# icyveins7/pydsproutines

Measured on AMD Instinct MI355X. Metric: CAF Msamples/s (4k template x 256 freq bins), higher is better.
Workload: dtype f32

## Files before the change

### pydsproutines_amd/csrc/caf_fused.hip

```cpp
#include <algorithm>
#include <cstdlib>
#include <type_traits>

#include "caf_internal.h"
#include "caf_fft_dev.h"
#include "caf_wave.h"

namespace caf {

constexpr int FB = 16384;
constexpr int FP_P1 = 4384;
constexpr int FP_IM = 16 * FP_P1;
constexpr int F_LDS_BYTES = 2 * FP_IM;
constexpr int F_LDS_DATA = F_LDS_BYTES / 8;
__host__ __device__ constexpr int fp_row2(int n2) { return ((n2 >> 1) & 3) * 1088 + ((n2 & 1) + 2 * (n2 >> 3)) * 256; }
static_assert(fp_row2(15) + 256 <= FP_P1 && FP_P1 % 256 == 32, "planar image geometry");

#define CAF_AS1 __attribute__((address_space(1)))
#define CAF_AS4 __attribute__((address_space(4)))
typedef float v2f_t __attribute__((ext_vector_type(2)));
typedef float v4f_t __attribute__((ext_vector_type(4)));
typedef int v2i_t __attribute__((ext_vector_type(2)));
__device__ __forceinline__ float2 ld2(const float2* base, uint32_t elem) {
    const uint64_t u = *reinterpret_cast<const CAF_AS1 uint64_t*>((const CAF_AS1 char*)base + (elem << 3));
// ... 96 lines not shown
__device__ __forceinline__ Tp* uniform_ptr(Tp* p) {
    const uint64_t v = reinterpret_cast<uint64_t>(p);
    const uint32_t lo = __builtin_amdgcn_readfirstlane((uint32_t)v);
    const uint32_t hi = __builtin_amdgcn_readfirstlane((uint32_t)(v >> 32));
    return reinterpret_cast<Tp*>(((uint64_t)hi << 32) | lo);
}
__device__ __forceinline__ __amdgpu_buffer_rsrc_t buf_of(const void* base, uint32_t bytes) {
    return __builtin_amdgcn_make_buffer_rsrc(const_cast<void*>(base), 0, (int)bytes, 0x00020000);
}
constexpr int CAF_AUX_SC1 = 16;
constexpr int CAF_AUX_NT = 2;
template <int MODE>
__device__ __forceinline__ void tile_store(__amdgpu_buffer_rsrc_t r, uint32_t voff, uint32_t soff, float val) {
    __builtin_amdgcn_raw_buffer_store_b32(__builtin_bit_cast(int, val), r, (int)voff, (int)soff, MODE == 1 ? (CAF_AUX_SC1 | CAF_AUX_NT) : 0);
}

struct F1Direct {
    float* out0;
    float* out1;
    const float* inv_e;
    const float* tscale;
    int64_t num_shifts;
    int32_t step, blk_abs;
    PeakRec* partial;
    int64_t ppt, shift_start;
};
template <int FT, int MODE = 0, int NV4 = 4, bool PK = false>
__device__ __forceinline__ void fused_item(float2* __restrict__ s_d, const float2* __restrict__ s_tw2,
                                           const float2* __restrict__ s_tw3,
                                           const float2* __restrict__ xb,
                                           const float2* __restrict__ hc,
                                           const int32_t* __restrict__ shifts,
                                           const float2* __restrict__ tw1,
                                           int32_t table_mode, int32_t nfreq, int32_t nhyp, int blk, int h0, int h1,
                                           int32_t tiles_per_blk, float* __restrict__ vt,
                                           int32_t* __restrict__ imax = nullptr, const F1Direct* f1 = nullptr) {
    static_assert(FT == 1024, "one radix-16 butterfly per thread and pass: 1024 threads (wave w owns plane n1 = w)");
    constexpr int BPT = 1;
    const int tid = threadIdx.x;
    const lds_char* img = (const lds_char*)s_d;
    const uint32_t img0 = __builtin_amdgcn_readfirstlane((uint32_t)(uintptr_t)img);
    const uint32_t wave_u = __builtin_amdgcn_readfirstlane((uint32_t)tid >> 6);
    const uint32_t m0_x1 = img0 + wave_u * 256u, m0_w = img0 + wave_u * (uint32_t)FP_P1;
    const uint32_t m2 = fp_m2((uint32_t)tid);
    constexpr int nv4 = NV4;
    float bv[16];
    uint32_t bi[4];
    float ge[16];
    if (MODE == 2 || MODE == 5) {
#pragma unroll
        for (int o = 0; o < 16; ++o) bv[o] = -1.f;
#pragma unroll
// ... 19 lines not shown
#pragma unroll
            for (int o = 0; o < 16; ++o) ge[o] = __builtin_sqrtf(ge[o]);
        }
    }

    uint32_t pk_d0 = 0, pk_nv = 0;
    if (PK) {
        const int n1 = tid & 15, n2 = (tid >> 4) & 15, q = tid >> 8;
        pk_d0 = (uint32_t)(((n2 >> 2) + 4 * q) * 64 + n1 + 16 * (n2 & 3));
        pk_nv = f1_bytes >> 2;
    }
    float2 w[BPT];
    const float2* xp = xb + (int64_t)blk * FB;
#pragma unroll
    for (int j = 0; j < BPT; ++j) w[j] = ld2(tw1, 1024u + m2);
    float* vt_blk = vt + (int64_t)blk * tiles_per_blk * nhyp * 64;
    const __amdgpu_buffer_rsrc_t rvt = buf_of(uniform_ptr(vt_blk), (uint32_t)tiles_per_blk * (uint32_t)nhyp * 256u);

    const float2* hrow_cur;
    uint32_t hb_cur;
    auto row_of = [&](int h) {
        if (table_mode) {
            hrow_cur = hc + (int64_t)h * FB;
            hb_cur = (uint32_t)tid;
        } else {
            const int t = h / nfreq;
            const int32_t sh = *((const CAF_AS4 int32_t*)shifts + (h - t * nfreq));
            hrow_cur = hc + (int64_t)t * FB;
            hb_cur = fp_hbase(m2, sh);
        }
    };
    float2 pr[BPT][16];
    float2 xr[BPT][16];
#pragma unroll
    for (int j = 0; j < BPT; ++j)
#pragma unroll
        for (int a = 0; a < 16; ++a) xr[j][a] = ld2(xp, 1024u * a + m2);
    row_of(h0);
#pragma unroll
    for (int j = 0; j < BPT; ++j)
#pragma unroll
        for (int a = 0; a < 16; ++a)
            pr[j][a] = cmul(xr[j][a],
                            ld2(hrow_cur, (1024u * a + hb_cur) & (FB - 1)));

    for (int h = h0; h < h1; ++h) {
        const bool more = h + 1 < h1;
        uint32_t hoff = (uint32_t)h * 256u;
        asm volatile("" : "+s"(hoff));
        int lz = 0;
        asm volatile("" : "+v"(lz));
        __amdgpu_buffer_rsrc_t f1_r0 = rvt, f1_r1 = rvt;
        float f1_ts = 0.f;
        if (MODE == 3) {
            f1_ts = *((const CAF_AS4 float*)f1->tscale + h);
            f1_r0 = buf_of(uniform_ptr(f1->out0 + (int64_t)h * f1->num_shifts + f1_rel0), f1->out0 ? f1_bytes : 0u);
            if (f1->out1)
                f1_r1 = buf_of(uniform_ptr(f1->out1 + (int64_t)h * f1->num_shifts + f1_rel0), f1_bytes);
        }
        float pk_v[4] = {-1.f, -1.f, -1.f, -1.f};
        uint32_t pk_i[4] = {0u, 0u, 0u, 0u};
        if (MODE == 4) {
            f1_ts = __builtin_sqrtf(*((const CAF_AS4 float*)f1->tscale + h / nfreq));
// ... 79 lines not shown
        __syncthreads();
#pragma unroll
        for (int j = 0; j < BPT; ++j) {
            const int idx = tid + j * FT;
            const int n1 = idx & 15, n2 = (idx >> 4) & 15, q = idx >> 8;
            const uint32_t rd4 = fp_rd4((uint32_t)idx), rd4i = fp_im(rd4);
            __builtin_amdgcn_sched_barrier(0);
            float2 pf0, pf1, pf2, pf3;
            if (MODE < 2) {
                lds_get4c(img, rd4, rd4i, pf0, pf1, pf2, pf3);
                __builtin_amdgcn_sched_barrier(0);
#pragma unroll
                for (int a = 0; a < 16; ++a) pr[j][a] = cmul(xr[j][a], hn[j][a]);
                __builtin_amdgcn_sched_barrier(0);
            }
#pragma unroll
            for (int i = 0; i < 4; ++i) {
                uint32_t lzi = 0;
                asm volatile("" : "+v"(lzi));
                float2 a0, a1, a2, a3;
                if (MODE < 2 && i == 0)
                    a0 = pf0, a1 = pf1, a2 = pf2, a3 = pf3;
                else
                    lds_get4c(img, rd4 + 1024u * i + lzi, rd4i + 1024u * i + lzi, a0, a1, a2, a3);
                const float2 s02 = cadd(a0, a2), d02 = csub(a0, a2), s13 = cadd(a1, a3), d13 = mulj(csub(a1, a3));
#pragma unroll
                for (int n4 = 0; n4 < 4; ++n4) {
                    if (n4 >= nv4) continue;
                    const float2 yq = n4 == 0 ? cadd(s02, s13) : n4 == 1 ? cadd(d02, d13) : n4 == 2 ? csub(s02, s13) : csub(d02, d13);
                    const int tile_u = 16 * i + 64 * n4;
// ... 24 lines not shown
                        const float gq = ge[4 * i + n4] * f1_ts;
                        const v2f_t ov = {yq.x * gq, yq.y * gq};
                        const uint32_t v3 = (uint32_t)(tile_t * 64 + n1 + 16 * (n2 & 3)) << 3, s3 = (uint32_t)tile_u * 512u;
                        __builtin_amdgcn_raw_buffer_store_b64(__builtin_bit_cast(v2i_t, ov), f1_r0, (int)v3, (int)s3, CAF_AUX_NT);
                    } else if (MODE == 3) {
                        const float outv = val * (ge[4 * i + n4] * f1_ts);
                        if (PK) {
                            const bool up = ((uint32_t)(pk_d0 + (16 * i + 64 * n4) * 64) < pk_nv) & (outv > pk_v[n4]);
                            pk_v[n4] = up ? outv : pk_v[n4];
                            pk_i[n4] = up ? (uint32_t)i : pk_i[n4];
                        }
                        const uint32_t v3 = (uint32_t)(tile_t * 64 + n1 + 16 * (n2 & 3)) << 2, s3 = (uint32_t)tile_u * 256u;
                        __builtin_amdgcn_raw_buffer_store_b32(__builtin_bit_cast(int, outv), f1_r0, (int)v3, (int)s3, CAF_AUX_NT);
                        if (f1->out1)
                            __builtin_amdgcn_raw_buffer_store_b32(__builtin_bit_cast(int, outv), f1_r1, (int)v3, (int)s3, CAF_AUX_NT);
                    } else {
                        tile_store<MODE>(rvt, voff, soff, val);
                    }
                }
                __builtin_amdgcn_sched_barrier(0);
            }
            if (MODE >= 2) {
#pragma unroll
                for (int a = 2 * EH; a < 16; ++a) pr[j][a] = cmul(xr[j][a], hn[j][a]);
            }
            __builtin_amdgcn_sched_barrier(0);
        }
        if (PK) {
            float bvv = pk_v[0];
            uint32_t bq = 0, bii = pk_i[0];
#pragma unroll
            for (int n4 = 1; n4 < NV4; ++n4) {
                const bool up = pk_v[n4] > bvv;
                bvv = up ? pk_v[n4] : bvv;
                bq = up ? (uint32_t)n4 : bq;
// ... 583 lines not shown
__device__ __forceinline__ int32_t pq_load(const int32_t* p) {
    return __hip_atomic_load(p, __ATOMIC_RELAXED, __HIP_MEMORY_SCOPE_AGENT);
}
__device__ __forceinline__ const CAF_AS4 PersistParams* params_of(const PersistParams* p) {
    uint64_t v = reinterpret_cast<uint64_t>(p);
    asm volatile("" : "+s"(v));
    return reinterpret_cast<const CAF_AS4 PersistParams*>(v);
}
typedef float v4f_u_t __attribute__((ext_vector_type(4), aligned(4)));
typedef int v4i_u_t __attribute__((ext_vector_type(4), aligned(4)));

constexpr int TW_H = 32;
constexpr int TW_PITCH = TW_H + 1;
constexpr int TW_LDS = 64 * TW_PITCH;

template <bool SURF, int DS>
__device__ __forceinline__ void transpose_wave(float* __restrict__ lds, const PersistParams* pp, int z, int tile0) {
    const CAF_AS4 PersistParams* P = params_of(pp);
    const int32_t ntmpl = P->ntmpl, nfreq = P->nfreq, step = P->step, tiles_per_blk = P->tiles_per_blk;
    const int64_t num_shifts = P->num_shifts, shift_start = P->shift_start;
    const int wave_id = __builtin_amdgcn_readfirstlane((int)(threadIdx.x >> 6));
    const int lane = threadIdx.x & 63;
    float* s_w = lds + wave_id * TW_LDS;
    const int tile = tile0 + wave_id;
    if (tile >= tiles_per_blk) return;
    const int blk = P->blk0 + z;
    const int sl0 = DS == 2 ? 128 * (tile & 255) + (tile >> 8) : tile * 64;
    const int64_t rel0 = (int64_t)blk * step + sl0;
    int64_t nv = num_shifts - (int64_t)blk * step;
    if (nv > step) nv = step;
    const int nrows = sl0 < nv ? (int)min((int64_t)64, (nv - sl0 + DS - 1) / DS) : 0;
    const int64_t pidx = (int64_t)blk * tiles_per_blk + tile;
    PeakRec* partial = P->partial;
    const int64_t ppt = P->partial_per_tmpl;
    const int s4 = 4 * (lane & 15), fq = lane >> 4;
    const int nsteps = (nfreq + TW_H - 1) / TW_H;
    for (int t = 0; t < ntmpl; ++t) {
        if (nrows == 0) {
            if (lane == 0 && partial) {
                PeakRec r;
                r.v = -1.f;
                r.delay = 0x7fffffff;
                r.f = 0;
                partial[(int64_t)t * ppt + pidx] = r;
            }
            continue;
        }
        const float* vin = uniform_ptr(P->vt + (((int64_t)z * tiles_per_blk + tile) * ntmpl + t) * (int64_t)nfreq * 64);
        float* srow0 = SURF ? uniform_ptr(P->surface + ((int64_t)t * num_shifts + rel0) * nfreq) : nullptr;
        const float ts = P->tscale[t];
        const __amdgpu_buffer_rsrc_t rin = buf_of(vin, (uint32_t)nfreq * 256u);
        const __amdgpu_buffer_rsrc_t rout = buf_of(srow0, (uint32_t)(((nrows - 1) * DS + 1) * nfreq) * 4u);
        const __amdgpu_buffer_rsrc_t rie = buf_of(uniform_ptr(P->inv_e + rel0), (uint32_t)((nrows - 1) * DS + 1) * 4u);
        float g[4], bv[4];
        int32_t bi[4];
#pragma unroll
        for (int k = 0; k < 4; ++k) {
            g[k] = __builtin_bit_cast(float, __builtin_amdgcn_raw_buffer_load_b32(rie, (s4 + k) * 4 * DS, 0, 0)) * ts;
            bv[k] = -1.f;
            bi[k] = 0;
        }
        v4f_t qa[TW_H / 4], qb[TW_H / 4];
        auto load_step = [&](v4f_t(&q)[TW_H / 4], int s) {
#pragma unroll
            for (int i = 0; i < TW_H / 4; ++i)
                q[i] = __builtin_bit_cast(v4f_t, __builtin_amdgcn_raw_buffer_load_b128(rin, (fq * 64 + s4) * 4,
                                                                                       (s * TW_H + 4 * i) * 256, CAF_AUX_SC1 | CAF_AUX_NT));
        };
        const int half = lane >> 5, col = lane & 31;
        const float* srd = s_w + half * TW_PITCH + col;
        float* swr = s_w + s4 * TW_PITCH + fq;
        const int voff = (half * DS * nfreq + col) * 4;
        auto do_step = [&](v4f_t(&q)[TW_H / 4], int s) {
            const int f0 = s * TW_H;
#pragma unroll
            for (int i = 0; i < TW_H / 4; ++i) {
                const int hyp = f0 + 4 * i + fq;
                const bool hv = hyp < nfreq;
                const float x[4] = {q[i].x * g[0], q[i].y * g[1], q[i].z * g[2], q[i].w * g[3]};
#pragma unroll
                for (int k = 0; k < 4; ++k) {
                    if (SURF) swr[k * TW_PITCH + 4 * i] = x[k];
                    const bool up = hv & (x[k] > bv[k]);
                    bv[k] = up ? x[k] : bv[k];
                    bi[k] = up ? hyp : bi[k];
                }
            }
            load_step(q, s + 2);
            if (SURF) {
                __builtin_amdgcn_wave_barrier();
                const int vo = (f0 + col < nfreq) ? voff : 0x7ffffff0;
#pragma unroll
                for (int r = 0; r < 64; r += 2)
                    __builtin_amdgcn_raw_buffer_store_b32(__builtin_bit_cast(int, srd[r * TW_PITCH]), rout, vo,
                                                          (r * DS * nfreq + f0) * 4, CAF_AUX_NT);
                __builtin_amdgcn_wave_barrier();
            }
        };
        load_step(qa, 0);
        load_step(qb, 1);
        for (int s = 0; s < nsteps; s += 2) {
            do_step(qa, s);
            do_step(qb, s + 1);
        }
#pragma unroll
        for (int k = 0; k < 4; ++k) wave_argmax<32, 16>(bv[k], bi[k]);
        float* row_max = P->row_max;
        int32_t* row_arg = P->row_arg;
        float best = -1.f;
        int32_t bdel = 0x7fffffff, bfrq = 0;
        if (fq == 0) {
            const int64_t o = (int64_t)t * num_shifts + rel0 + s4 * DS;
#pragma unroll
            for (int k = 0; k < 4; ++k) {
                if (s4 + k < nrows) {
                    if (row_max) row_max[o + k * DS] = bv[k] < 0.f ? __builtin_nanf("") : bv[k];
                    if (row_arg) row_arg[o + k * DS] = bi[k];
                    if (bv[k] > best) {
                        best = bv[k];
                        bdel = s4 + k;
                        bfrq = bi[k];
                    }
                }
            }
        }
        if (partial) {
            wave_argmax<8>(best, bdel, bfrq);
            if (lane == 0) {
                PeakRec r;
                r.v = best;
                r.delay = (int32_t)(shift_start + rel0 + bdel * DS);
                r.f = bfrq;
                partial[(int64_t)t * ppt + pidx] = r;
            }
        }
// ... 196 lines not shown
    for (;;) {
        const CAF_AS4 PersistParams* P = params_of(pp);
        const int ipb = P->ipb;
        const int z = item / ipb;
        if (P->nosurf)
            reduce_wave_nosurf(pp, z, (item - z * ipb) * PQ_TILES);
        else if (P->dstride == 2) {
            if (P->nfreq == 1)
                transpose_wave_f1<2>(pp, z, (item - z * ipb) * PQ_TILES);
            else if (P->surface)
                transpose_wave<true, 2>(lds, pp, z, (item - z * ipb) * PQ_TILES);
            else
                transpose_wave<false, 2>(lds, pp, z, (item - z * ipb) * PQ_TILES);
        } else if (P->nfreq == 1)
            transpose_wave_f1<1>(pp, z, (item - z * ipb) * PQ_TILES);
        else if (P->surface)
            transpose_wave<true, 1>(lds, pp, z, (item - z * ipb) * PQ_TILES);
        else
            transpose_wave<false, 1>(lds, pp, z, (item - z * ipb) * PQ_TILES);
        if (wave_id == 0) {
            int32_t* pq = P->pq;
            const int n_fft = P->n_fft, n_tr = P->n_tr, ngroups = P->ngroups;
            int next = -1;
            const int t = __builtin_amdgcn_readfirstlane(pq_load(&pq[PQ_TR_NEXT]));
            if (t < n_tr) {
                const bool fft_left = __builtin_amdgcn_readfirstlane(pq_load(&pq[PQ_FFT_NEXT])) < n_fft;
                if (!fft_left || __builtin_amdgcn_readfirstlane(pq_load(&pq[PQ_DONE + t / ipb])) >= ngroups) {
                    int my = 0;
                    if (lane0) my = atomicAdd(&pq[PQ_TR_NEXT], 1);
                    my = __builtin_amdgcn_readfirstlane(my);
                    if (my < n_tr) {
// ... 69 lines not shown
        f1.partial = nullptr;
        f1.ppt = 0;
        f1.shift_start = 0;
        f1.inv_e = P->inv_e;
        f1.tscale = P->tscale;
        f1.num_shifts = P->num_shifts;
        f1.step = P->step;
        f1.blk_abs = P->blk0 + blk;
        const int64_t o = ((int64_t)blk * ngroups + grp) * P->tiles_per_blk * 64;
        fused_item<1024, 5, NV4>((float2*)s_d, (const float2*)s_tw2, (const float2*)s_tw3, P->xb, P->hc, P->shifts, P->tw1,
                                 P->table_mode, P->nfreq, nhyp, blk, h0, h1, P->tiles_per_blk, P->vmax + o, P->imax + o, &f1);
    } else if (KIND == 1) {
        const int64_t o = ((int64_t)blk * ngroups + grp) * P->tiles_per_blk * 64;
        fused_item<1024, 2, NV4>((float2*)s_d, (const float2*)s_tw2, (const float2*)s_tw3, P->xb, P->hc, P->shifts, P->tw1,
                            P->table_mode, P->nfreq, nhyp, blk, h0, h1, P->tiles_per_blk, P->vmax + o, P->imax + o);
    } else {
        fused_item<1024, 1, NV4>((float2*)s_d, (const float2*)s_tw2, (const float2*)s_tw3, P->xb, P->hc, P->shifts, P->tw1,
                            P->table_mode, P->nfreq, nhyp, blk, h0, h1, P->tiles_per_blk, P->vt);
    }
    __builtin_amdgcn_fence(__ATOMIC_RELEASE, "workgroup");
    __syncthreads();
    if (threadIdx.x == 0)
        __hip_atomic_fetch_add(&params_of(pp)->pq[PQ_DONE + blk], 1, __ATOMIC_RELAXED, __HIP_MEMORY_SCOPE_AGENT);
}

__device__ __forceinline__ void cq_params(const CAF_AS4 PersistParams* P, int blk, F1Direct& f1) {
    f1.out0 = P->cqf;
    f1.out1 = nullptr;
    f1.partial = nullptr;
    f1.ppt = 0;
// ... 175 lines not shown
                }
#undef CAF_FFT_ROLE2F
            } else if (__builtin_amdgcn_readfirstlane(params_of(pp)->block_log2) == 15) {
                const int tpb2 = __builtin_amdgcn_readfirstlane(params_of(pp)->tiles_per_blk);
                const bool cq = params_of(pp)->cqf != nullptr;
#define CAF_FFT_ROLE2(NN, CC) persistent_fft_item2<NN, CC>((lds_float2*)s_d, (const lds_float2*)s_tw2, (const lds_float2*)s_tw3, pp, item)
                if (tpb2 <= 256) { if (cq) CAF_FFT_ROLE2(0, true); else CAF_FFT_ROLE2(0, false); }
                else if (tpb2 <= 384) { if (cq) CAF_FFT_ROLE2(2, true); else CAF_FFT_ROLE2(2, false); }
                else { if (cq) CAF_FFT_ROLE2(4, true); else CAF_FFT_ROLE2(4, false); }
#undef CAF_FFT_ROLE2
            }
            else {
                const int kind3 = params_of(pp)->cqf ? 3
                                  : params_of(pp)->surface_t ? 5
                                  : __builtin_amdgcn_readfirstlane(params_of(pp)->f1_direct) ? (params_of(pp)->partial ? 4 : 2)
                                  : __builtin_amdgcn_readfirstlane(params_of(pp)->nosurf) ? 1 : 0;
                const int tpb = __builtin_amdgcn_readfirstlane(params_of(pp)->tiles_per_blk);
#define CAF_FFT_ROLE(K, Q) persistent_fft_item<K, Q>((lds_float2*)s_d, (const lds_float2*)s_tw2, (const lds_float2*)s_tw3, pp, item)
                if (tpb <= 128) {
                    if (kind3 == 5) CAF_FFT_ROLE(5, 2); else if (kind3 == 4) CAF_FFT_ROLE(4, 2); else if (kind3 == 3) CAF_FFT_ROLE(3, 2); else if (kind3 == 2) CAF_FFT_ROLE(2, 2); else if (kind3 == 1) CAF_FFT_ROLE(1, 2); else CAF_FFT_ROLE(0, 2);
                } else if (tpb <= 192) {
                    if (kind3 == 5) CAF_FFT_ROLE(5, 3); else if (kind3 == 4) CAF_FFT_ROLE(4, 3); else if (kind3 == 3) CAF_FFT_ROLE(3, 3); else if (kind3 == 2) CAF_FFT_ROLE(2, 3); else if (kind3 == 1) CAF_FFT_ROLE(1, 3); else CAF_FFT_ROLE(0, 3);
                } else {
                    if (kind3 == 5) CAF_FFT_ROLE(5, 4); else if (kind3 == 4) CAF_FFT_ROLE(4, 4); else if (kind3 == 3) CAF_FFT_ROLE(3, 4); else if (kind3 == 2) CAF_FFT_ROLE(2, 4); else if (kind3 == 1) CAF_FFT_ROLE(1, 4); else CAF_FFT_ROLE(0, 4);
                }
#undef CAF_FFT_ROLE
            }
            if (STATS) {
                const uint64_t now = wall_clock64();
                t_fft += (uint32_t)(now - tmark);
                tmark = now;
                ++c_fft;
            }
        } else {
            persistent_tile_run((lds_float*)s_d, (lds_int*)&s_cmd[1], pp, item);
            if (STATS) {
                const uint64_t now = wall_clock64();
                t_tile += (uint32_t)(now - tmark);
                tmark = now;
// ... 65 lines not shown
```

### pydsproutines_amd/csrc/caf_internal.h

```cpp
#pragma once
#include <hip/hip_runtime.h>
#include <stdint.h>

#include "caf.h"
#include "caf_energy.h"

#include <map>
#include <mutex>
#include <string>
#include <utility>
#include <vector>

namespace caf {

constexpr int MUL_THREADS = 256;
constexpr int MAG_THREADS = 256;
constexpr int MAG_S = 64;
constexpr int MAG_F = 128;

inline int64_t energy_prefix_doubles(int64_t m) { return ((m + 2) & ~(int64_t)1) + (m + 63) / 64 + 1; }

struct PeakRec {
    float v;
    int32_t delay;
// ... 194 lines not shown
                            int64_t nb, int64_t L, int64_t B, int32_t ntaps, float2* rows, hipStream_t st);
void launch_fos_taps_pad(const float* taps, int32_t ntaps, int64_t B, float2* row, hipStream_t st);
void launch_fos_scatter(const float2* rows, int64_t b0, int64_t nb, int64_t L, int64_t B, int32_t ntaps, int32_t dsr,
                        int32_t phase, float2* out, int64_t nout, hipStream_t st);

void launch_parity_major(const float2* in, float2* out, int64_t rows, int32_t half, hipStream_t st, bool butterfly = false);
void launch_parity_pairs(const float2* in, float2* out, int64_t rows, int32_t quarter, hipStream_t st);
void launch_fused_caf(const float2* xb, const float2* hc, const int32_t* shifts, const float2* tw1,
                      const float2* tw23, int32_t table_mode, int32_t nfreq, int32_t nhyp, int32_t hyp_per_wg,
                      int32_t nblk, int32_t tiles_per_blk, float* vt, hipStream_t st);
void launch_transpose_norm_argmax(const float* vt, int32_t ntmpl, int32_t nfreq, const float* tscale,
                                  const float* inv_e, int64_t num_shifts, int64_t shift_start, int32_t step,
                                  int32_t blk0, int32_t nblk, int32_t tiles_per_blk, float* surface, float* row_max,
                                  int32_t* row_arg, PeakRec* partial, int64_t partial_per_tmpl, hipStream_t st);

struct PersistParams {
    const float2* xb;
    const float2* hc;
    const int32_t* shifts;
    const float2* tw1;
    const float2* tw23;
    float* vt;
    int32_t table_mode, nfreq, nhyp, hyp_per_wg, nblk, tiles_per_blk;
    int32_t block_log2;
    int32_t dstride;
    int32_t npart;
    int32_t ntmpl, step, blk0;
    int32_t gpt;
    const float* tscale;
    const float* inv_e;
    int64_t num_shifts, shift_start;
    float* surface;
    float* row_max;
    int32_t* row_arg;
    PeakRec* partial;
    int64_t partial_per_tmpl;
    int32_t* pq;
    int32_t tr_slots, ngroups, n_fft, ipb, n_tr;
    int32_t nosurf;
    int32_t f1_direct;
    float* cqf;
    float* surface_t;
    float* vmax;
    int32_t* imax;
    int32_t* dbg;
};
void launch_butterfly_order(const float2* in, float2* out, int64_t nchunks, hipStream_t st);
void launch_caf_persistent(const PersistParams* h, PersistParams* d_params, int32_t n_wgs, hipStream_t st);

struct FftPlan {
    void* plan = nullptr;
    void* info = nullptr;
    void* work = nullptr;
    size_t work_bytes = 0;
    int exec(void* in, void* out, hipStream_t st);
    void* slot = nullptr;
    hipEvent_t last_use = nullptr;
    bool last_use_pending = false;

// ... 20 lines not shown
```

### pydsproutines_amd/csrc/caf_plan.hip

```cpp
#include <algorithm>
#include <cmath>
#include <complex>
#include <cstring>
#include <mutex>
#include <vector>

#include <unistd.h>

#include "caf_internal.h"

namespace caf {

static thread_local std::string g_last_error;
void set_error(const std::string& msg) { g_last_error = msg; }

}

using namespace caf;

static int env_int(const char* name, int dflt, bool* is_set = nullptr) {
    const char* e = getenv(name);
    if (is_set) *is_set = e != nullptr;
    return e ? atoi(e) : dflt;
}
// ... 501 lines not shown
        hpw = best;
    }
    if (p->B == 65536 && !forced) hpw = std::min(hpw, p->npart >= 6 ? 8 : p->npart > 1 ? 16 : 32);
    if (F % hpw != 0)
        for (int dv = hpw; dv >= std::max(4, hpw / 3); --dv)
            if (F % dv == 0) return dv;
    return hpw;
}

static int nosurf_groups_per_tmpl(const caf_plan_t* p) {
    if (!p->persistent || p->B != 16384 || p->F < p->hyp_per_wg) return 0;
    const int gpt = (p->F + p->hyp_per_wg - 1) / p->hyp_per_wg;
    return 2 * (int64_t)gpt <= p->F ? gpt : 0;
}
static bool writes_surface_t(const caf_plan_t* p) { return p->persistent && p->B == 16384; }
static int64_t vt_floats(const caf_plan_t* p, int64_t blocks, int64_t rows) { return blocks * p->tiles_per_blk * rows * 64; }

static void build_batch(caf_plan p, const Build& b) {
    const int T = p->T, F = p->F;
    int nb = b.d->blocks_per_batch;
    if (nb <= 0) {
        if (p->fused) {
            const int64_t per_block = vt_floats(p, 1, (int64_t)T * F) * 4;
            nb = (int)std::max<int64_t>(1, std::min<int64_t>(65535, ((int64_t)18 << 30) / per_block));
        } else {
            const int64_t per_block = (int64_t)T * F * p->pitch * 8;
            nb = (int)std::max<int64_t>(1, std::min<int64_t>(64, ((int64_t)128 << 20) / per_block));
        }
    }
    nb = (int)std::min<int64_t>(nb, std::max<int64_t>(1, b.total_blocks));
    p->nb = nb;
    p->max_blocks = (b.total_blocks + nb - 1) / nb * nb;
    p->partial_per_tmpl = p->max_blocks * p->tiles_per_blk;
    p->hyp_per_wg = choose_hyp_per_wg(p, b);
    p->nb_nosurf = nb;
    if (const int64_t gpt = nosurf_groups_per_tmpl(p)) {
        const int64_t cap = (int64_t)nb * F / (2 * gpt);
        p->nb_nosurf = (int)std::max<int64_t>(nb, std::min<int64_t>(std::min<int64_t>(cap, 4096), std::max<int64_t>(1, b.total_blocks)));
    }
}

static int32_t build_buffers(caf_plan p, const Build& b) {
    const int T = p->T, F = p->F, NP = p->npart;
    const int64_t B = p->B, max_rx = b.d->max_rx_len;
    int rc;
    if ((rc = p->alloc(&p->d_hc, b.nspec * B))) return rc;
    if ((rc = p->alloc(&p->d_shifts, std::max(F, 1)))) return rc;
    if ((rc = p->alloc(&p->d_tscale, T))) return rc;
// ... 229 lines not shown
    const float2* rx = nullptr;
    int64_t rx_len = 0, shift_start = 0, num_shifts = 0;
    int64_t nblk = 0, nblk_pad = 0;
    bool want_peak = false;
    hipStream_t st = nullptr;
};

struct PersistMode {
    int gpt = 0;
    int nosurf = 0;
    int hyp_per_wg = 0;
    int ngroups = 0;
    int nb_launch = 0;
    int64_t imax_off = 0;
    bool f1_direct = false, f1_item_peaks = false, cqf_rows = false;
};

static int32_t decide_mode(const caf_plan_t* p, Call* c, PersistMode* m) {
    const int T = p->T, F = p->F;
    if (c->d_surface_t && F == 1) {
        CAF_REQUIRE(!c->d_surface, "d_surface and d_surface_t cannot both be given");
        c->d_surface = c->d_surface_t;
        c->d_surface_t = nullptr;
    }
    const bool surf_t = c->d_surface_t != nullptr;
    CAF_REQUIRE(!surf_t || (writes_surface_t(p) && !c->d_surface && !c->d_cqf),
                "the hypothesis-major surface (d_surface_t) is written by the persistent engine with 16384-point blocks (templates of "
                "at most 8192 samples), and not together with d_surface or d_cqf");
    if (!p->fused) return CAF_OK;
    m->cqf_rows = c->d_cqf != nullptr;
// ... 7 lines not shown
            const int g2 = (m->gpt + 1) / 2;
            if ((F + g2 - 1) / g2 > 256 || (int64_t)T * g2 * blocks_launch < (int64_t)40 * p->n_cus) break;
            m->gpt = g2;
        }
    }
    if (surf_t) m->gpt = (F + p->hyp_per_wg - 1) / p->hyp_per_wg;
    CAF_REQUIRE(m->gpt || (int64_t)(p->B / 64) * T * F * 256 < ((int64_t)1 << 32),
                "too many hypotheses (templates x frequencies) for one launch with |y|^2 tiles: ask for no surface, "
                "or split the templates over several plans");
    static const bool f1_env = env_int("CAF_PERSIST_F1DIRECT", 1) != 0;
    static const bool f1_pk_env = env_int("CAF_F1_ITEM_PEAKS", 1) != 0;
    m->f1_direct = p->persistent && p->B == 16384 && F == 1 && f1_env && !m->cqf_rows &&
                   (c->d_row_max || c->d_surface || (c->want_peak && f1_pk_env));
    m->f1_item_peaks = m->f1_direct && c->want_peak && f1_pk_env;
    m->nosurf = !m->gpt ? 0 : surf_t ? 2 : 1;
    m->hyp_per_wg = m->gpt ? (F + m->gpt - 1) / m->gpt : p->hyp_per_wg;
    m->ngroups = m->gpt ? T * m->gpt : (T * F + p->hyp_per_wg - 1) / p->hyp_per_wg;
    m->nb_launch = m->gpt ? p->nb_nosurf : p->nb;
    m->imax_off = vt_floats(p, m->nb_launch, m->ngroups);
    if (p->B == 65536) m->ngroups *= 2;
    return CAF_OK;
}

static int32_t run_direct(caf_plan p, const Call& c) {
    CAF_REQUIRE(!c.d_cqf, "the direct engine has no complex-QF output (create the plan with CAF_ENGINE_ROCFFT)");
    p->stage_begin(3, c.st);
    launch_direct_caf(c.rx, c.shift_start, c.num_shifts, p->T, p->F, p->dir_k, p->d_dir_pos, p->d_dir_w, p->d_tscale, c.d_surface,
                      c.d_row_max, c.d_row_arg, c.want_peak ? p->d_partial : nullptr, p->partial_per_tmpl, c.st);
    p->stage_end(c.st);
    return CAF_OK;
// ... 71 lines not shown
    h.blk0 = (int32_t)b0;
    h.gpt = m.gpt;
    h.tscale = p->d_tscale;
    h.inv_e = p->d_inv_e;
    h.num_shifts = c.num_shifts;
    h.shift_start = c.shift_start;
    h.surface = c.d_surface;
    h.row_max = c.d_row_max;
    h.row_arg = c.d_row_arg;
    h.partial = c.want_peak && (!m.f1_direct || m.f1_item_peaks) ? p->d_partial : nullptr;
    h.partial_per_tmpl = p->partial_per_tmpl;
    h.pq = p->d_pq;
    h.tr_slots = p->tr_slots;
    h.ngroups = m.ngroups;
    h.n_fft = nbk * m.ngroups;
    h.ipb = (p->tiles_per_blk + 15) / 16;
    h.n_tr = m.f1_direct || m.cqf_rows ? 0 : nbk * h.ipb;
    h.nosurf = m.nosurf;
    h.f1_direct = m.f1_direct ? 1 : 0;
    h.cqf = c.d_cqf;
    h.surface_t = c.d_surface_t;
    h.vmax = p->d_vt;
    h.imax = reinterpret_cast<int32_t*>(p->d_vt + m.imax_off);
    return h;
}

static void persist_report(caf_plan p, const PersistParams& h, const int32_t* h_dbg, bool surface, hipStream_t st) {
    hipEvent_t ev;
    (void)hipEventCreate(&ev);
    (void)hipEventRecord(ev, st);
    bool done = false;
// ... 6 lines not shown
        _exit(3);
    }
    std::vector<int32_t> q(4 + h.nblk);
    (void)hipMemcpy(q.data(), p->d_pq, q.size() * 4, hipMemcpyDeviceToHost);
    double sum[2][5] = {{0}};
    int cnt[2] = {0, 0};
    uint32_t t0 = 0xffffffffu, t1 = 0, tl = 0;
    for (int w = 0; w < p->n_cus; ++w) {
        const int pref = ((w >> 3) & 31) >= 32 - p->tr_slots;
        ++cnt[pref];
        for (int k = 0; k < 5; ++k) sum[pref][k] += h_dbg[8 * w + k];
        t0 = std::min(t0, (uint32_t)h_dbg[8 * w + 5]);
        tl = std::max(tl, (uint32_t)h_dbg[8 * w + 5]);
        t1 = std::max(t1, (uint32_t)h_dbg[8 * w + 6]);
    }
    fprintf(stderr, "[caf persistent] n_fft=%d n_tr=%d | fft_next=%d tr_next=%d watchdog=%d,%d | first start -> last end "
            "%.0f us, last start +%.0f us\n", h.n_fft, h.n_tr, q[0], q[1], q[2], q[3], (t1 - t0) / 100.0, (tl - t0) / 100.0);
    for (int r = 0; r < 2; ++r)
        if (cnt[r])
            fprintf(stderr,
                    "  %s workgroups (%d): claim+wait %.0f us, fft %.0f us in %.1f items (%.1f us each), tiles %.0f us "
                    "in %.1f items (%.1f us each)\n",
                    r ? "tile-first" : "fft-first", cnt[r], sum[r][0] / cnt[r] / 100.0, sum[r][1] / cnt[r] / 100.0,
                    sum[r][3] / cnt[r], sum[r][3] > 0 ? sum[r][1] / sum[r][3] / 100.0 : 0.0,
                    sum[r][2] / cnt[r] / 100.0, sum[r][4] / cnt[r],
                    sum[r][4] > 0 ? sum[r][2] / sum[r][4] / 100.0 : 0.0);
    const char* lst = getenv("CAF_PERSIST_TILE_ONLY");
    if (!lst) return;
    PersistParams h2 = h;
    h2.n_fft = 0;
    h2.ngroups = 0;
    h2.dbg = nullptr;
// ... 91 lines not shown
        const bool want_mag = c.d_surface || c.d_row_max || c.d_row_arg || c.want_peak;
        p->stage_begin(5, st);
        if (want_mag)
            launch_magsq(p->d_pbuf, p->pitch, T, F, p->d_tscale, p->d_inv_e, c.num_shifts, c.shift_start, p->step, (int32_t)b0,
                         p->nb, p->tiles_per_blk, c.d_surface, c.d_row_max, c.d_row_arg,
                         c.want_peak ? p->d_partial : nullptr, p->partial_per_tmpl, st);
        p->stage_end(st);
    }
    return CAF_OK;
}

static void reduce_peaks(caf_plan p, const PersistMode& m, const Call& c) {
    hipStream_t st = c.st;
    p->stage_begin(6, st);
    int64_t nrec = p->direct ? (c.num_shifts + 127) / 128 : (p->fused ? c.nblk : c.nblk_pad) * p->tiles_per_blk;
    if (m.f1_item_peaks) {
        nrec = c.nblk * 16;
    } else if (m.f1_direct) {
        launch_rows_peak(c.d_row_max ? c.d_row_max : c.d_surface, p->T, c.num_shifts, c.shift_start, p->d_partial,
                         p->partial_per_tmpl, st);
        nrec = rows_peak_chunks(c.num_shifts);
    }
    launch_peak_reduce(p->d_partial, nrec, p->partial_per_tmpl, p->T, p->d_partial + (int64_t)p->T * p->partial_per_tmpl,
                       c.d_peak_val, c.d_peak_delay, c.d_peak_freq, st);
    p->stage_end(st);
}

int32_t caf_plan_execute2(caf_plan p, const float* d_rx, int64_t rx_len, int64_t shift_start, int64_t num_shifts,
                          const caf_outputs2* out2, void* stream) {
    CAF_REQUIRE(p && d_rx && out2, "caf_plan_execute: NULL argument");
// ... 74 lines not shown
```

Baseline: 1263.

## Store FFT tile output as quad records with 128-bit writes in persistent path

```diff
diff --git a/pydsproutines_amd/csrc/caf_fused.hip b/pydsproutines_amd/csrc/caf_fused.hip
--- a/pydsproutines_amd/csrc/caf_fused.hip
+++ b/pydsproutines_amd/csrc/caf_fused.hip
@@ -134,6 +134,12 @@
 __device__ __forceinline__ void tile_store(__amdgpu_buffer_rsrc_t r, uint32_t voff, uint32_t soff, float val) {
     __builtin_amdgcn_raw_buffer_store_b32(__builtin_bit_cast(int, val), r, (int)voff, (int)soff, MODE == 1 ? (CAF_AUX_SC1 | CAF_AUX_NT) : 0);
 }
+typedef uint32_t v4u_t __attribute__((ext_vector_type(4)));
+__device__ __forceinline__ void quad_store(__amdgpu_buffer_rsrc_t r, uint32_t voff, uint32_t soff, float v0, float v1, float v2, float v3) {
+    const v4u_t v = {__builtin_bit_cast(uint32_t, v0), __builtin_bit_cast(uint32_t, v1), __builtin_bit_cast(uint32_t, v2),
+                     __builtin_bit_cast(uint32_t, v3)};
+    __builtin_amdgcn_raw_buffer_store_b128(v, r, (int)voff, (int)soff, CAF_AUX_SC1 | CAF_AUX_NT);
+}
 
 struct F1Direct {
     float* out0;
@@ -145,7 +151,7 @@
     PeakRec* partial;
     int64_t ppt, shift_start;
 };
-template <int FT, int MODE = 0, int NV4 = 4, bool PK = false>
+template <int FT, int MODE = 0, int NV4 = 4, bool PK = false, bool QUAD = false>
 __device__ __forceinline__ void fused_item(float2* __restrict__ s_d, const float2* __restrict__ s_tw2,
                                            const float2* __restrict__ s_tw3,
                                            const float2* __restrict__ xb,
@@ -156,6 +162,7 @@
                                            int32_t tiles_per_blk, float* __restrict__ vt,
                                            int32_t* __restrict__ imax = nullptr, const F1Direct* f1 = nullptr) {
     static_assert(FT == 1024, "one radix-16 butterfly per thread and pass: 1024 threads (wave w owns plane n1 = w)");
+    static_assert(!QUAD || MODE == 1, "quad-tile records: the write-through tile mode only");
     constexpr int BPT = 1;
     const int tid = threadIdx.x;
     const lds_char* img = (const lds_char*)s_d;
@@ -205,8 +212,9 @@
     const float2* xp = xb + (int64_t)blk * FB;
 #pragma unroll
     for (int j = 0; j < BPT; ++j) w[j] = ld2(tw1, 1024u + m2);
-    float* vt_blk = vt + (int64_t)blk * tiles_per_blk * nhyp * 64;
-    const __amdgpu_buffer_rsrc_t rvt = buf_of(uniform_ptr(vt_blk), (uint32_t)tiles_per_blk * (uint32_t)nhyp * 256u);
+    const int32_t vt_tiles = QUAD ? 4 * quad_records(tiles_per_blk) : tiles_per_blk;
+    float* vt_blk = vt + (int64_t)blk * vt_tiles * nhyp * 64;
+    const __amdgpu_buffer_rsrc_t rvt = buf_of(uniform_ptr(vt_blk), (uint32_t)vt_tiles * (uint32_t)nhyp * 256u);
 
     const float2* hrow_cur;
     uint32_t hb_cur;
@@ -237,7 +245,7 @@
 
     for (int h = h0; h < h1; ++h) {
         const bool more = h + 1 < h1;
-        uint32_t hoff = (uint32_t)h * 256u;
+        uint32_t hoff = (uint32_t)h * (QUAD ? 1024u : 256u);
         asm volatile("" : "+s"(hoff));
         int lz = 0;
         asm volatile("" : "+v"(lz));
@@ -347,6 +355,7 @@
                 for (int a = 0; a < 16; ++a) pr[j][a] = cmul(xr[j][a], hn[j][a]);
                 __builtin_amdgcn_sched_barrier(0);
             }
+            float qv[4][4];
 #pragma unroll
             for (int i = 0; i < 4; ++i) {
                 uint32_t lzi = 0;
@@ -401,11 +410,19 @@
                         __builtin_amdgcn_raw_buffer_store_b32(__builtin_bit_cast(int, outv), f1_r0, (int)v3, (int)s3, CAF_AUX_NT);
                         if (f1->out1)
                             __builtin_amdgcn_raw_buffer_store_b32(__builtin_bit_cast(int, outv), f1_r1, (int)v3, (int)s3, CAF_AUX_NT);
+                    } else if (QUAD) {
+                        qv[n4][i] = val;
                     } else {
                         tile_store<MODE>(rvt, voff, soff, val);
                     }
                 }
                 __builtin_amdgcn_sched_barrier(0);
+            }
+            if (QUAD) {
+                const uint32_t voff = ((uint32_t)((n2 >> 2) + 4 * q) * (uint32_t)nhyp * 256u + (uint32_t)(n1 + 16 * (n2 & 3)) * 4u) << 2;
+#pragma unroll
+                for (int n4 = 0; n4 < nv4; ++n4)
+                    quad_store(rvt, voff, (uint32_t)(16 * n4) * (uint32_t)nhyp * 1024u + hoff, qv[n4][0], qv[n4][1], qv[n4][2], qv[n4][3]);
             }
             if (MODE >= 2) {
 #pragma unroll
@@ -1019,10 +1036,13 @@
 constexpr int TW_PITCH = TW_H + 1;
 constexpr int TW_LDS = 64 * TW_PITCH;
 
-template <bool SURF, int DS>
+template <bool SURF, int DS, bool QUAD = false>
 __device__ __forceinline__ void transpose_wave(float* __restrict__ lds, const PersistParams* pp, int z, int tile0) {
+    static_assert(!QUAD || DS == 1, "quad-tile records: the 16384-point role only");
+    constexpr int DK = QUAD ? 1024 : DS;
     const CAF_AS4 PersistParams* P = params_of(pp);
-    const int32_t ntmpl = P->ntmpl, nfreq = P->nfreq, step = P->step, tiles_per_blk = P->tiles_per_blk;
+    const int32_t ntmpl = P->ntmpl, nfreq = P->nfreq, step = P->step;
+    const int32_t tiles_per_blk = QUAD ? 4 * quad_records(P->tiles_per_blk) : P->tiles_per_blk;
     const int64_t num_shifts = P->num_shifts, shift_start = P->shift_start;
     const int wave_id = __builtin_amdgcn_readfirstlane((int)(threadIdx.x >> 6));
     const int lane = threadIdx.x & 63;
@@ -1030,15 +1050,18 @@
     const int tile = tile0 + wave_id;
     if (tile >= tiles_per_blk) return;
     const int blk = P->blk0 + z;
-    const int sl0 = DS == 2 ? 128 * (tile & 255) + (tile >> 8) : tile * 64;
+    const int sl0 = QUAD      ? 64 * ((tile >> 2) & 15) + 4096 * (tile >> 6) + 16 * (tile & 3)
+                    : DS == 2 ? 128 * (tile & 255) + (tile >> 8)
+                              : tile * 64;
     const int64_t rel0 = (int64_t)blk * step + sl0;
     int64_t nv = num_shifts - (int64_t)blk * step;
     if (nv > step) nv = step;
-    const int nrows = sl0 < nv ? (int)min((int64_t)64, (nv - sl0 + DS - 1) / DS) : 0;
+    const int nrows = sl0 >= nv ? 0 : QUAD ? (int)min((int64_t)(3 * DK + 16), nv - sl0) : (int)min((int64_t)64, (nv - sl0 + DS - 1) / DS);
     const int64_t pidx = (int64_t)blk * tiles_per_blk + tile;
     PeakRec* partial = P->partial;
     const int64_t ppt = P->partial_per_tmpl;
     const int s4 = 4 * (lane & 15), fq = lane >> 4;
+    const int d4 = QUAD ? (lane & 15) : s4;
     const int nsteps = (nfreq + TW_H - 1) / TW_H;
     for (int t = 0; t < ntmpl; ++t) {
         if (nrows == 0) {
@@ -1051,31 +1074,34 @@
             }
             continue;
         }
-        const float* vin = uniform_ptr(P->vt + (((int64_t)z * tiles_per_blk + tile) * ntmpl + t) * (int64_t)nfreq * 64);
+        const float* vin = QUAD ? uniform_ptr(P->vt + ((((int64_t)z * tiles_per_blk + tile) >> 2) * ntmpl + t) * (int64_t)nfreq * 256)
+                                : uniform_ptr(P->vt + (((int64_t)z * tiles_per_blk + tile) * ntmpl + t) * (int64_t)nfreq * 64);
         float* srow0 = SURF ? uniform_ptr(P->surface + ((int64_t)t * num_shifts + rel0) * nfreq) : nullptr;
         const float ts = P->tscale[t];
-        const __amdgpu_buffer_rsrc_t rin = buf_of(vin, (uint32_t)nfreq * 256u);
-        const __amdgpu_buffer_rsrc_t rout = buf_of(srow0, (uint32_t)(((nrows - 1) * DS + 1) * nfreq) * 4u);
-        const __amdgpu_buffer_rsrc_t rie = buf_of(uniform_ptr(P->inv_e + rel0), (uint32_t)((nrows - 1) * DS + 1) * 4u);
+        constexpr int HB = QUAD ? 1024 : 256;
+        const uint32_t ext = QUAD ? (uint32_t)nrows : (uint32_t)((nrows - 1) * DS + 1);
+        const __amdgpu_buffer_rsrc_t rin = buf_of(vin, (uint32_t)nfreq * (uint32_t)HB);
+        const __amdgpu_buffer_rsrc_t rout = buf_of(srow0, (ext * (uint32_t)nfreq) * 4u);
+        const __amdgpu_buffer_rsrc_t rie = buf_of(uniform_ptr(P->inv_e + rel0), ext * 4u);
         float g[4], bv[4];
         int32_t bi[4];
 #pragma unroll
         for (int k = 0; k < 4; ++k) {
-            g[k] = __builtin_bit_cast(float, __builtin_amdgcn_raw_buffer_load_b32(rie, (s4 + k) * 4 * DS, 0, 0)) * ts;
+            g[k] = __builtin_bit_cast(float, __builtin_amdgcn_raw_buffer_load_b32(rie, QUAD ? (d4 + k * DK) * 4 : (s4 + k) * 4 * DS, 0, 0)) * ts;
             bv[k] = -1.f;
             bi[k] = 0;
         }
         v4f_t qa[TW_H / 4], qb[TW_H / 4];
+        const int ldv = QUAD ? fq * HB + (16 * (tile & 3) + d4) * 16 : (fq * 64 + s4) * 4;
         auto load_step = [&](v4f_t(&q)[TW_H / 4], int s) {
 #pragma unroll
             for (int i = 0; i < TW_H / 4; ++i)
-                q[i] = __builtin_bit_cast(v4f_t, __builtin_amdgcn_raw_buffer_load_b128(rin, (fq * 64 + s4) * 4,
-                                                                                       (s * TW_H + 4 * i) * 256, CAF_AUX_SC1 | CAF_AUX_NT));
+                q[i] = __builtin_bit_cast(v4f_t, __builtin_amdgcn_raw_buffer_load_b128(rin, ldv, (s * TW_H + 4 * i) * HB, CAF_AUX_SC1 | CAF_AUX_NT));
         };
         const int half = lane >> 5, col = lane & 31;
         const float* srd = s_w + half * TW_PITCH + col;
         float* swr = s_w + s4 * TW_PITCH + fq;
-        const int voff = (half * DS * nfreq + col) * 4;
+        const int voff = (half * DK * nfreq + col) * 4;
         auto do_step = [&](v4f_t(&q)[TW_H / 4], int s) {
             const int f0 = s * TW_H;
 #pragma unroll
@@ -1098,7 +1124,7 @@
 #pragma unroll
                 for (int r = 0; r < 64; r += 2)
                     __builtin_amdgcn_raw_buffer_store_b32(__builtin_bit_cast(int, srd[r * TW_PITCH]), rout, vo,
-                                                          (r * DS * nfreq + f0) * 4, CAF_AUX_NT);
+                                                          ((QUAD ? (r & 3) * DK + (r >> 2) : r * DS) * nfreq + f0) * 4, CAF_AUX_NT);
                 __builtin_amdgcn_wave_barrier();
             }
         };
@@ -1115,15 +1141,15 @@
         float best = -1.f;
         int32_t bdel = 0x7fffffff, bfrq = 0;
         if (fq == 0) {
-            const int64_t o = (int64_t)t * num_shifts + rel0 + s4 * DS;
+            const int64_t o = (int64_t)t * num_shifts + rel0 + d4 * DS;
 #pragma unroll
             for (int k = 0; k < 4; ++k) {
-                if (s4 + k < nrows) {
-                    if (row_max) row_max[o + k * DS] = bv[k] < 0.f ? __builtin_nanf("") : bv[k];
-                    if (row_arg) row_arg[o + k * DS] = bi[k];
+                if (d4 + k * (QUAD ? DK : 1) < nrows) {
+                    if (row_max) row_max[o + k * DK] = bv[k] < 0.f ? __builtin_nanf("") : bv[k];
+                    if (row_arg) row_arg[o + k * DK] = bi[k];
                     if (bv[k] > best) {
                         best = bv[k];
-                        bdel = s4 + k;
+                        bdel = d4 + k * (QUAD ? DK : 1);
                         bfrq = bi[k];
                     }
                 }
@@ -1350,7 +1376,12 @@
                 transpose_wave<false, 2>(lds, pp, z, (item - z * ipb) * PQ_TILES);
         } else if (P->nfreq == 1)
             transpose_wave_f1<1>(pp, z, (item - z * ipb) * PQ_TILES);
-        else if (P->surface)
+        else if (P->quad) {
+            if (P->surface)
+                transpose_wave<true, 1, true>(lds, pp, z, (item - z * ipb) * PQ_TILES);
+            else
+                transpose_wave<false, 1, true>(lds, pp, z, (item - z * ipb) * PQ_TILES);
+        } else if (P->surface)
             transpose_wave<true, 1>(lds, pp, z, (item - z * ipb) * PQ_TILES);
         else
             transpose_wave<false, 1>(lds, pp, z, (item - z * ipb) * PQ_TILES);
@@ -1450,6 +1481,9 @@
         const int64_t o = ((int64_t)blk * ngroups + grp) * P->tiles_per_blk * 64;
         fused_item<1024, 2, NV4>((float2*)s_d, (const float2*)s_tw2, (const float2*)s_tw3, P->xb, P->hc, P->shifts, P->tw1,
                             P->table_mode, P->nfreq, nhyp, blk, h0, h1, P->tiles_per_blk, P->vmax + o, P->imax + o);
+    } else if (KIND == 6) {
+        fused_item<1024, 1, NV4, false, true>((float2*)s_d, (const float2*)s_tw2, (const float2*)s_tw3, P->xb, P->hc, P->shifts, P->tw1,
+                                              P->table_mode, P->nfreq, nhyp, blk, h0, h1, P->tiles_per_blk, P->vt);
     } else {
         fused_item<1024, 1, NV4>((float2*)s_d, (const float2*)s_tw2, (const float2*)s_tw3, P->xb, P->hc, P->shifts, P->tw1,
                             P->table_mode, P->nfreq, nhyp, blk, h0, h1, P->tiles_per_blk, P->vt);
@@ -1655,15 +1689,16 @@
                 const int kind3 = params_of(pp)->cqf ? 3
                                   : params_of(pp)->surface_t ? 5
                                   : __builtin_amdgcn_readfirstlane(params_of(pp)->f1_direct) ? (params_of(pp)->partial ? 4 : 2)
-                                  : __builtin_amdgcn_readfirstlane(params_of(pp)->nosurf) ? 1 : 0;
+                                  : __builtin_amdgcn_readfirstlane(params_of(pp)->nosurf) ? 1
+                                  : __builtin_amdgcn_readfirstlane(params_of(pp)->quad) ? 6 : 0;
                 const int tpb = __builtin_amdgcn_readfirstlane(params_of(pp)->tiles_per_blk);
 #define CAF_FFT_ROLE(K, Q) persistent_fft_item<K, Q>((lds_float2*)s_d, (const lds_float2*)s_tw2, (const lds_float2*)s_tw3, pp, item)
                 if (tpb <= 128) {
-                    if (kind3 == 5) CAF_FFT_ROLE(5, 2); else if (kind3 == 4) CAF_FFT_ROLE(4, 2); else if (kind3 == 3) CAF_FFT_ROLE(3, 2); else if (kind3 == 2) CAF_FFT_ROLE(2, 2); else if (kind3 == 1) CAF_FFT_ROLE(1, 2); else CAF_FFT_ROLE(0, 2);
+                    if (kind3 == 5) CAF_FFT_ROLE(5, 2); else if (kind3 == 4) CAF_FFT_ROLE(4, 2); else if (kind3 == 3) CAF_FFT_ROLE(3, 2); else if (kind3 == 2) CAF_FFT_ROLE(2, 2); else if (kind3 == 1) CAF_FFT_ROLE(1, 2); else if (kind3 == 6) CAF_FFT_ROLE(6, 2); else CAF_FFT_ROLE(0, 2);
                 } else if (tpb <= 192) {
-                    if (kind3 == 5) CAF_FFT_ROLE(5, 3); else if (kind3 == 4) CAF_FFT_ROLE(4, 3); else if (kind3 == 3) CAF_FFT_ROLE(3, 3); else if (kind3 == 2) CAF_FFT_ROLE(2, 3); else if (kind3 == 1) CAF_FFT_ROLE(1, 3); else CAF_FFT_ROLE(0, 3);
+                    if (kind3 == 5) CAF_FFT_ROLE(5, 3); else if (kind3 == 4) CAF_FFT_ROLE(4, 3); else if (kind3 == 3) CAF_FFT_ROLE(3, 3); else if (kind3 == 2) CAF_FFT_ROLE(2, 3); else if (kind3 == 1) CAF_FFT_ROLE(1, 3); else if (kind3 == 6) CAF_FFT_ROLE(6, 3); else CAF_FFT_ROLE(0, 3);
                 } else {
-                    if (kind3 == 5) CAF_FFT_ROLE(5, 4); else if (kind3 == 4) CAF_FFT_ROLE(4, 4); else if (kind3 == 3) CAF_FFT_ROLE(3, 4); else if (kind3 == 2) CAF_FFT_ROLE(2, 4); else if (kind3 == 1) CAF_FFT_ROLE(1, 4); else CAF_FFT_ROLE(0, 4);
+                    if (kind3 == 5) CAF_FFT_ROLE(5, 4); else if (kind3 == 4) CAF_FFT_ROLE(4, 4); else if (kind3 == 3) CAF_FFT_ROLE(3, 4); else if (kind3 == 2) CAF_FFT_ROLE(2, 4); else if (kind3 == 1) CAF_FFT_ROLE(1, 4); else if (kind3 == 6) CAF_FFT_ROLE(6, 4); else CAF_FFT_ROLE(0, 4);
                 }
 #undef CAF_FFT_ROLE
             }
diff --git a/pydsproutines_amd/csrc/caf_internal.h b/pydsproutines_amd/csrc/caf_internal.h
--- a/pydsproutines_amd/csrc/caf_internal.h
+++ b/pydsproutines_amd/csrc/caf_internal.h
@@ -232,6 +232,10 @@
                                   int32_t blk0, int32_t nblk, int32_t tiles_per_blk, float* surface, float* row_max,
                                   int32_t* row_arg, PeakRec* partial, int64_t partial_per_tmpl, hipStream_t st);
 
+__host__ __device__ constexpr int32_t quad_records(int32_t tiles_per_blk) {
+    return 16 * (tiles_per_blk >> 6) + ((tiles_per_blk & 63) < 16 ? (tiles_per_blk & 63) : 16);
+}
+
 struct PersistParams {
     const float2* xb;
     const float2* hc;
@@ -261,6 +265,7 @@
     float* surface_t;
     float* vmax;
     int32_t* imax;
+    int32_t quad;
     int32_t* dbg;
 };
 void launch_butterfly_order(const float2* in, float2* out, int64_t nchunks, hipStream_t st);
diff --git a/pydsproutines_amd/csrc/caf_plan.hip b/pydsproutines_amd/csrc/caf_plan.hip
--- a/pydsproutines_amd/csrc/caf_plan.hip
+++ b/pydsproutines_amd/csrc/caf_plan.hip
@@ -539,7 +539,9 @@
     return 2 * (int64_t)gpt <= p->F ? gpt : 0;
 }
 static bool writes_surface_t(const caf_plan_t* p) { return p->persistent && p->B == 16384; }
-static int64_t vt_floats(const caf_plan_t* p, int64_t blocks, int64_t rows) { return blocks * p->tiles_per_blk * rows * 64; }
+static bool quad_capable(const caf_plan_t* p) { return p->persistent && p->B == 16384; }
+static int64_t tiles_alloc(const caf_plan_t* p) { return quad_capable(p) ? 4 * quad_records(p->tiles_per_blk) : p->tiles_per_blk; }
+static int64_t vt_floats(const caf_plan_t* p, int64_t blocks, int64_t rows) { return blocks * tiles_alloc(p) * rows * 64; }
 
 static void build_batch(caf_plan p, const Build& b) {
     const int T = p->T, F = p->F;
@@ -556,7 +558,7 @@
     nb = (int)std::min<int64_t>(nb, std::max<int64_t>(1, b.total_blocks));
     p->nb = nb;
     p->max_blocks = (b.total_blocks + nb - 1) / nb * nb;
-    p->partial_per_tmpl = p->max_blocks * p->tiles_per_blk;
+    p->partial_per_tmpl = p->max_blocks * tiles_alloc(p);
     p->hyp_per_wg = choose_hyp_per_wg(p, b);
     p->nb_nosurf = nb;
     if (const int64_t gpt = nosurf_groups_per_tmpl(p)) {
@@ -816,6 +818,7 @@
     int nb_launch = 0;
     int64_t imax_off = 0;
     bool f1_direct = false, f1_item_peaks = false, cqf_rows = false;
+    bool quad = false;
 };
 
 static int32_t decide_mode(const caf_plan_t* p, Call* c, PersistMode* m) {
@@ -853,6 +856,7 @@
                    (c->d_row_max || c->d_surface || (c->want_peak && f1_pk_env));
     m->f1_item_peaks = m->f1_direct && c->want_peak && f1_pk_env;
     m->nosurf = !m->gpt ? 0 : surf_t ? 2 : 1;
+    m->quad = quad_capable(p) && !m->nosurf && !m->f1_direct && !m->cqf_rows && F > 1 && env_int("CAF_PERSIST_QUAD", 1) != 0;
     m->hyp_per_wg = m->gpt ? (F + m->gpt - 1) / m->gpt : p->hyp_per_wg;
     m->ngroups = m->gpt ? T * m->gpt : (T * F + p->hyp_per_wg - 1) / p->hyp_per_wg;
     m->nb_launch = m->gpt ? p->nb_nosurf : p->nb;
@@ -954,7 +958,8 @@
     h.tr_slots = p->tr_slots;
     h.ngroups = m.ngroups;
     h.n_fft = nbk * m.ngroups;
-    h.ipb = (p->tiles_per_blk + 15) / 16;
+    h.quad = m.quad ? 1 : 0;
+    h.ipb = m.quad ? (quad_records(p->tiles_per_blk) + 3) / 4 : (p->tiles_per_blk + 15) / 16;
     h.n_tr = m.f1_direct || m.cqf_rows ? 0 : nbk * h.ipb;
     h.nosurf = m.nosurf;
     h.f1_direct = m.f1_direct ? 1 : 0;
@@ -991,8 +996,8 @@
         tl = std::max(tl, (uint32_t)h_dbg[8 * w + 5]);
         t1 = std::max(t1, (uint32_t)h_dbg[8 * w + 6]);
     }
-    fprintf(stderr, "[caf persistent] n_fft=%d n_tr=%d | fft_next=%d tr_next=%d watchdog=%d,%d | first start -> last end "
-            "%.0f us, last start +%.0f us\n", h.n_fft, h.n_tr, q[0], q[1], q[2], q[3], (t1 - t0) / 100.0, (tl - t0) / 100.0);
+    fprintf(stderr, "[caf persistent] n_fft=%d n_tr=%d quad=%d | fft_next=%d tr_next=%d watchdog=%d,%d | first start -> last end "
+            "%.0f us, last start +%.0f us\n", h.n_fft, h.n_tr, h.quad, q[0], q[1], q[2], q[3], (t1 - t0) / 100.0, (tl - t0) / 100.0);
     for (int r = 0; r < 2; ++r)
         if (cnt[r])
             fprintf(stderr,
@@ -1114,6 +1119,7 @@
     hipStream_t st = c.st;
     p->stage_begin(6, st);
     int64_t nrec = p->direct ? (c.num_shifts + 127) / 128 : (p->fused ? c.nblk : c.nblk_pad) * p->tiles_per_blk;
+    if (m.quad) nrec = c.nblk * 4 * quad_records(p->tiles_per_blk);
     if (m.f1_item_peaks) {
         nrec = c.nblk * 16;
     } else if (m.f1_direct) {
```

Result: no change. 1267, median of 6 (+0.3%).
